# kai-neumann/OrthoSfM

Measured on AMD Instinct MI355X. Metric: image-pairs matched/sec + BA iterations/sec (N images, M tracks) at 1/2/4/8 GPU, higher is better.
Workload: dtype i8; 1 GPU; 50 orthographic images, 20000 SIFT features/img, exhaustive matching (1225 pairs, low-res gate + two-way + cross-check + lists; SURVEY 8d's unit of work: up to, not including, RANSAC-F -- the pass through RANSAC-F is `with_geometric_verification`); views=50, features_per_view=20000, pairs=1225

## Files before the change

### orthosfm_amd/csrc/match_all.hip

```cpp
#include <algorithm>
#include <chrono>
#include <cstdlib>
#include <cstring>

#include "match_internal.h"
#include "ransac_kernels.h"
#include "ransac_affine.h"

namespace osfm {

namespace {

struct Lap {
    std::chrono::steady_clock::time_point t_chunk = std::chrono::steady_clock::now();
    void operator()(const char *what) const
    {
        static const bool trace = getenv("OSFM_MATCH_TRACE") != nullptr;
        if (trace) fprintf(stderr, "[osfm match] %-18s %9.3f ms\n", what,
            std::chrono::duration<double, std::milli>(std::chrono::steady_clock::now() - t_chunk).count());
    }
};

struct ChunkLists {
    std::vector<int64_t> m12_off, corr_off;
    std::vector<int32_t> len12;
    std::vector<uint8_t> keep;
};

int compact_chunk(osfm_matcher *m, const ChunkLists &h, int n, int64_t chunk_corr, int32_t *corr, int64_t written, int *chunk_no)
{
    const osfm_match_options &o = m->opts;
    hipStream_t s = m->stream;
    OSFM_RETURN_IF(m->d_m12_off.reserve(n * 8));
    OSFM_RETURN_IF(m->d_corr_off.reserve(n * 8));
    OSFM_RETURN_IF(m->d_len12.reserve(n * 4));
    OSFM_RETURN_IF(m->d_keep_pair.reserve(n));
    const int cb = o.geometric_verification ? 0 : ((*chunk_no)++ & 1);
    DeviceBuffer &dcorr = cb ? m->d_corr_alt : m->d_corr;
    if (m->copied_used[cb]) OSFM_HIP_CHECK(hipEventSynchronize(m->ev_copied[cb]));
    OSFM_RETURN_IF(dcorr.reserve((size_t)chunk_corr * 8));
    OSFM_HIP_CHECK(hipMemcpyAsync(m->d_m12_off.ptr, h.m12_off.data(), n * 8, hipMemcpyHostToDevice, s));
    OSFM_HIP_CHECK(hipMemcpyAsync(m->d_corr_off.ptr, h.corr_off.data(), n * 8, hipMemcpyHostToDevice, s));
    OSFM_HIP_CHECK(hipMemcpyAsync(m->d_len12.ptr, h.len12.data(), n * 4, hipMemcpyHostToDevice, s));
    OSFM_HIP_CHECK(hipMemcpyAsync(m->d_keep_pair.ptr, h.keep.data(), n, hipMemcpyHostToDevice, s));
    launch_compact_pairs(n, m->out.as<int32_t>(), m->d_m12_off.as<int64_t>(),
        m->d_len12.as<int32_t>(), m->d_corr_off.as<int64_t>(), m->d_keep_pair.as<uint8_t>(),
        dcorr.as<int32_t>(), s);
    OSFM_HIP_CHECK(hipGetLastError());
    if (!o.geometric_verification) {
        OSFM_HIP_CHECK(hipEventRecord(m->ev_compact[cb], s));
        OSFM_HIP_CHECK(hipStreamWaitEvent(m->copy_stream, m->ev_compact[cb], 0));
        OSFM_HIP_CHECK(hipMemcpyAsync(corr + 2 * written, dcorr.ptr, (size_t)chunk_corr * 8,
            hipMemcpyDeviceToHost, m->copy_stream));
        OSFM_HIP_CHECK(hipEventRecord(m->ev_copied[cb], m->copy_stream));
        m->copied_used[cb] = true;
    }
    return OSFM_OK;
}

int verify_chunk(osfm_matcher *m, const osfm_pair *pairs, const int *idx, int n, const std::vector<int32_t> &counts,
    const ChunkLists &h, int64_t chunk_corr, osfm_pair_result *results, int32_t *corr, int64_t capacity,
    int64_t *written_out, bool *overflow, const Lap &lap)
{
    const osfm_match_options &o = m->opts;
    hipStream_t s = m->stream;
    std::vector<RansacJob> jobs;
    std::vector<int> job_pair;
    OSFM_RETURN_IF(m->d_inl.reserve((size_t)chunk_corr * 4));
    OSFM_RETURN_IF(m->d_inl_count.reserve((size_t)n * 4));
    for (int k = 0; k < n; ++k) {
        if (!h.keep[k]) continue;
        const int p = idx[k];
        const ViewData &a = m->views[pairs[p].view_1], &b = m->views[pairs[p].view_2];
        if (a.n_positions < 0 || b.n_positions < 0) {
            set_error("match_all: geometric verification needs osfm_match_set_positions for views %d and %d",
                pairs[p].view_1, pairs[p].view_2);
            return OSFM_E_STATE;
        }
        RansacJob j;
        memset(&j, 0, sizeof(j));
        j.pos1 = a.positions.as<float>(); j.pos2 = b.positions.as<float>();
        j.corr = m->d_corr.as<int32_t>() + 2 * h.corr_off[k];
        j.k = counts[k];
        const int64_t hi = std::max(pairs[p].view_1, pairs[p].view_2), lo = std::min(pairs[p].view_1, pairs[p].view_2);
// ... 81 lines not shown
        if (o.use_lowres_matching && np1 * np2 > 1000000) lowres_idx.push_back(p);
        else full_idx.push_back(p);
    }

    {
        const int bs = batch_size_for(m->views, o, true);
        std::vector<osfm_pair> chunk;
        for (size_t start = 0; start < lowres_idx.size(); start += bs) {
            const size_t end = std::min(lowres_idx.size(), start + bs);
            chunk.clear();
            for (size_t k = start; k < end; ++k) chunk.push_back(pairs[lowres_idx[k]]);
            BatchResult res;
            BatchMode mode;
            mode.limit = o.num_lowres_features; mode.lowres = true; mode.apply = false;
            OSFM_RETURN_IF(run_batch(m, chunk.data(), (int)chunk.size(), mode, &res));
            for (size_t k = start; k < end; ++k) {
                const int p = lowres_idx[k];
                results[p].lowres_matches = res.counts[k - start];
                if (res.counts[k - start] < o.min_lowres_matches)
                    results[p].status = OSFM_PAIR_REJECTED_LOWRES;
                else
                    full_idx.push_back(p);
            }
        }
        std::sort(full_idx.begin(), full_idx.end());
    }
    if (phase == kPhaseGate) { if (total) *total = 0; return OSFM_OK; }

    const int min_matches = std::max(8, o.min_feature_matches);
    int64_t written = 0, written_out = 0;
    bool overflow = false;
    {
        const int bs = full_batch_size(m->views, o, full_idx.size());
        int chunk_no = 0;
        std::vector<osfm_pair> chunk;
        ChunkLists h;
        for (size_t start = 0; start < full_idx.size(); start += bs) {
            const size_t end = std::min(full_idx.size(), start + bs);
            const int n = (int)(end - start);
            chunk.clear();
            for (size_t k = start; k < end; ++k) chunk.push_back(pairs[full_idx[k]]);
            const Lap lap{};
            BatchResult res;
            BatchMode full_mode;
            if (m->expect_pairs > 0)
                full_mode.expect = std::min<int>(full_batch_size(m->views, o, (size_t)m->expect_pairs), m->expect_pairs);
            OSFM_RETURN_IF(run_batch(m, chunk.data(), n, full_mode, &res));
            lap("matched");
            h.m12_off.assign(n, 0); h.corr_off.assign(n, 0); h.len12.assign(n, 0); h.keep.assign(n, 0);
            int64_t chunk_corr = 0;
            for (int k = 0; k < n; ++k) {
                const int p = full_idx[start + k];
                osfm_pair_result &r = results[p];
                r.num_matches = res.counts[k];
                if (res.counts[k] < min_matches) { r.status = OSFM_PAIR_REJECTED_COUNT; continue; }
                r.status = OSFM_PAIR_MATCHED;
                r.offset = written + chunk_corr;
                h.keep[k] = 1;
                h.m12_off[k] = res.plans[k].off12;
                h.len12[k] = res.plans[k].len12;
                h.corr_off[k] = chunk_corr;
                chunk_corr += res.counts[k];
            }
            if (!o.geometric_verification && written + chunk_corr > capacity) overflow = true;
            if (chunk_corr > 0 && (o.geometric_verification || !overflow))
                OSFM_RETURN_IF(compact_chunk(m, h, n, chunk_corr, corr, written, &chunk_no));
            if (o.geometric_verification && chunk_corr > 0)
                OSFM_RETURN_IF(verify_chunk(m, pairs, full_idx.data() + start, n, res.counts, h, chunk_corr, results, corr,
                    capacity, &written_out, &overflow, lap));
            written += chunk_corr;
        }
    }
    if (!o.geometric_verification) OSFM_HIP_CHECK(hipStreamSynchronize(m->copy_stream));
    if (o.geometric_verification) written = written_out;
    if (total) *total = written;
    if (overflow) {
        set_error("match_all: %lld correspondences need more than the given capacity %lld",
            (long long)written, (long long)capacity);
        return OSFM_E_CAPACITY;
    }
    return OSFM_OK;
}

}
```

### orthosfm_amd/csrc/match_batch.hip

```cpp
#include <algorithm>
#include <cstdlib>
#include <cstring>

#include "match_internal.h"
#include "cashash_kernels.h"

namespace osfm {

int check_view(const osfm_matcher *m, int v, const char *what) { return check_view(m->views, v, what); }

void reset_stats(osfm_matcher *m) { memset(&m->stats, 0, sizeof(m->stats)); }

int run_batch(osfm_matcher *m, const osfm_pair *pairs, int num_pairs, const BatchMode &mode,
    BatchResult *res)
{
    const bool cascade = cascade_batch(m->opts, mode);
    if (cascade) OSFM_RETURN_IF(ensure_cashash(m));
    static const int forced_seg_tiles = [] { const char *e = getenv("OSFM_SEG_TILES"); return e ? atoi(e) : 0; }();
    const char *rescan_env = getenv("OSFM_FINISH_RESCAN");
    PlanKnobs knobs;
    knobs.seg_tiles = forced_seg_tiles;
    knobs.rescan_wave = rescan_env && strcmp(rescan_env, "wave") == 0;
    BatchPlan &plan = m->plan;
    res->counts.assign(num_pairs, 0);
    OSFM_RETURN_IF(plan_batch(m->views, m->opts, m->special_max, knobs, pairs, num_pairs, mode, &plan));
    res->plans = plan.plans;
    res->out_ints = plan.out_ints;
    const std::vector<PairPlan> &plans = plan.plans;
    std::vector<MatchProblem> *probs = plan.probs;
    const std::vector<SpecialJob> &spjobs = plan.spjobs, &spjobs_wide = plan.spjobs_wide;
    const int64_t out_ints = plan.out_ints, total_queries = plan.total_queries, rs_buckets = plan.rs_buckets;
    const int *total_blocks = plan.total_blocks, *max_n = plan.max_n;

    double grow = 1.0;
    if (mode.expect > num_pairs && num_pairs > 0) grow = 1.02 * (double)mode.expect / num_pairs;
    auto grown = [&](int64_t n) { return (size_t)((double)std::max<int64_t>(n, 1) * std::max(grow, 1.0)); };
    OSFM_RETURN_IF(m->out.reserve(grown(std::max<int64_t>(out_ints, 4)) * 4));
    OSFM_RETURN_IF(m->rowparts.reserve(grown(plan.rowpart_recs) * sizeof(RowPart)));
    OSFM_RETURN_IF(m->colparts.reserve(grown(plan.colpart_recs) * sizeof(ColPart)));
    OSFM_RETURN_IF(m->keep.reserve(grown(std::max<int64_t>(plan.keep_bytes, 16))));
    OSFM_RETURN_IF(m->exact_items.reserve(grown(total_queries) * sizeof(ExactItem)));
    OSFM_RETURN_IF(m->exact_count.reserve(16));
    if (plan.bucketed) {
        OSFM_RETURN_IF(m->rs_count.reserve(grown(rs_buckets) * sizeof(int32_t)));
        OSFM_RETURN_IF(m->rs_items.reserve(grown(plan.rs_items) * sizeof(RescoreItem)));
    }
    OSFM_RETURN_IF(m->sp_parts.reserve((size_t)std::max<int64_t>(plan.sp_recs, 1) * sizeof(RowPart)));
    hipStream_t s = m->stream;
    {
        std::vector<uint8_t> seen(m->views.size(), 0);
        for (int p = 0; p < num_pairs; ++p)
            for (int v : {plans[p].v1, plans[p].v2})
                if (!seen[v]) { seen[v] = 1; if (m->views[v].ready) OSFM_HIP_CHECK(hipStreamWaitEvent(s, m->views[v].ready, 0)); }
    }
    OSFM_RETURN_IF(m->sp_col.reserve((size_t)std::max<int64_t>(plan.sp_cols, 1) * 4));
    OSFM_RETURN_IF(m->d_spjobs.reserve(std::max<size_t>(spjobs.size() + spjobs_wide.size(), 1) * sizeof(SpecialJob)));
    if (!spjobs.empty())
        OSFM_HIP_CHECK(hipMemcpyAsync(m->d_spjobs.ptr, spjobs.data(), spjobs.size() * sizeof(SpecialJob),
            hipMemcpyHostToDevice, s));
    if (!spjobs_wide.empty())
        OSFM_HIP_CHECK(hipMemcpyAsync(m->d_spjobs.as<SpecialJob>() + spjobs.size(), spjobs_wide.data(),
            spjobs_wide.size() * sizeof(SpecialJob), hipMemcpyHostToDevice, s));
    int32_t *d_out = m->out.as<int32_t>();
    OSFM_HIP_CHECK(hipMemsetAsync(d_out, 0xff, (size_t)std::max<int64_t>(out_ints, 4) * 4, s));

    OSFM_HIP_CHECK(hipMemsetAsync(m->exact_count.ptr, 0, 16, s));
    bool timed[2] = {false, false};
    bool probed = false;
    for (int type = 0; type < 2; ++type) {
        const int np = (int)probs[type].size();
        if (np == 0) continue;
        for (int i = 0; i < np; ++i) {
            probs[type][i].m12 = d_out + plan.m12_off[type][i];
            probs[type][i].m21 = d_out + plan.m21_off[type][i];
        }
        OSFM_RETURN_IF(m->d_problems[type].reserve(np * sizeof(MatchProblem)));
        OSFM_RETURN_IF(m->mark_off[type].reserve(np * 2 * sizeof(int64_t)));
        OSFM_RETURN_IF(m->counts[type].reserve(np * sizeof(int32_t)));
        OSFM_HIP_CHECK(hipMemcpyAsync(m->d_problems[type].ptr, probs[type].data(),
            np * sizeof(MatchProblem), hipMemcpyHostToDevice, s));
        OSFM_HIP_CHECK(hipMemcpyAsync(m->mark_off[type].ptr, plan.mark_off[type].data(),
            np * 2 * sizeof(int64_t), hipMemcpyHostToDevice, s));
        OSFM_HIP_CHECK(hipMemsetAsync(m->counts[type].ptr, 0, np * sizeof(int32_t), s));
        const MatchProblem *dp = m->d_problems[type].as<MatchProblem>();
        const LoweTable tab = type == 0 ? m->tab_sift : m->tab_surf;
        const int ecap = (int)std::min<int64_t>(total_queries, 0x7fffffff);
        int32_t *ecount = m->exact_count.as<int32_t>() + type;

        if (cascade) {
            OSFM_HIP_CHECK(hipEventRecord(m->ev[type][0], s));
            timed[type] = true;
            OSFM_RETURN_IF(m->cas_state.reserve((size_t)std::max<int64_t>(plan.cas_queries[type], 1) * kCasMaxCand * 4));
            launch_cashash_match(type == 0 ? 128 : 64, dp, np, max_n[type], m->cas_state.as<int32_t>(), tab, s);
            OSFM_HIP_CHECK(hipEventRecord(m->ev[type][1], s));
        } else {
            if (total_blocks[type] > 0) { OSFM_HIP_CHECK(hipEventRecord(m->ev[type][0], s)); timed[type] = true; }
            unsigned long long *probe = nullptr;
            if (type == 0 && mode.limit == 0) {
                OSFM_RETURN_IF(m->clock_probe.reserve(16));
                OSFM_HIP_CHECK(hipMemsetAsync(m->clock_probe.ptr, 0, 16, s));
                probe = m->clock_probe.as<unsigned long long>();
                probed = true;
            }
            if (!m->zero_tile.ptr) {
                OSFM_RETURN_IF(m->zero_tile.reserve((size_t)kTileCols * 128));
                OSFM_HIP_CHECK(hipMemsetAsync(m->zero_tile.ptr, 0, (size_t)kTileCols * 128, s));
            }
            launch_match_tiles(type == 0 ? 8 : 4, plan.needs_mask[type], plan.any_special[type], plan.any_c0[type],
                plan.any_corrected[type], dp, np, total_blocks[type],
                m->rowparts.as<RowPart>(), m->colparts.as<ColPart>(), s, probe, m->zero_tile.as<int8_t>());
            if (timed[type]) OSFM_HIP_CHECK(hipEventRecord(m->ev[type][1], s));
            if (type == 0 && !(spjobs.empty() && spjobs_wide.empty())) {
                OSFM_HIP_CHECK(hipEventRecord(m->ev_sp[0], s));
                launch_match_special(dp, m->d_spjobs.as<SpecialJob>(), (int)spjobs.size(), m->sp_parts.as<RowPart>(),
                    m->sp_col.as<int32_t>(), s);
                launch_match_special_wide(dp, m->d_spjobs.as<SpecialJob>() + spjobs.size(), (int)spjobs_wide.size(),
                    m->sp_parts.as<RowPart>(), m->sp_col.as<int32_t>(), s);
                OSFM_HIP_CHECK(hipEventRecord(m->ev_sp[1], s));
            }
            const bool rs = type == 0 && plan.bucketed;
            if (rs) OSFM_HIP_CHECK(hipMemsetAsync(m->rs_count.ptr, 0, (size_t)rs_buckets * sizeof(int32_t), s));
            launch_match_finish(dp, np, max_n[type], m->rowparts.as<RowPart>(),
                m->colparts.as<ColPart>(), m->sp_parts.as<RowPart>(), m->sp_col.as<int32_t>(), tab, 0,
                m->exact_items.as<ExactItem>(), ecount, ecap, rs ? m->rs_count.as<int32_t>() : nullptr,
                rs ? m->rs_items.as<RescoreItem>() : nullptr, s);
            if (rs)
                launch_match_rescore(dp, np, m->rs_count.as<int32_t>(), m->rs_items.as<RescoreItem>(), rs_buckets, tab,
                    m->exact_items.as<ExactItem>(), ecount, ecap, s);
            launch_exact_scan(type == 0 ? 128 : 64, dp, m->exact_items.as<ExactItem>(), ecount, ecap,
                tab, s);
        }
        launch_cross_check_mark(dp, np, max_n[type], m->keep.as<uint8_t>(), m->keep.as<uint8_t>(),
            m->mark_off[type].as<int64_t>(), m->counts[type].as<int32_t>(), s);
        if (mode.apply)
            launch_cross_check_apply(dp, np, max_n[type], m->keep.as<uint8_t>(),
                m->keep.as<uint8_t>(), m->mark_off[type].as<int64_t>(), s);
        OSFM_HIP_CHECK(hipGetLastError());
    }

    std::vector<int32_t> hc[2];
    int32_t hexact[4] = {0, 0, 0, 0};
    for (int type = 0; type < 2; ++type) {
        hc[type].resize(probs[type].size());
        if (!hc[type].empty())
            OSFM_HIP_CHECK(hipMemcpyAsync(hc[type].data(), m->counts[type].ptr,
                hc[type].size() * sizeof(int32_t), hipMemcpyDeviceToHost, s));
    }
    OSFM_HIP_CHECK(hipMemcpyAsync(hexact, m->exact_count.ptr, 16, hipMemcpyDeviceToHost, s));
    unsigned long long hprobe[2] = {0, 0};
    if (probed) OSFM_HIP_CHECK(hipMemcpyAsync(hprobe, m->clock_probe.ptr, 16, hipMemcpyDeviceToHost, s));
    OSFM_HIP_CHECK(hipStreamSynchronize(s));
    m->stats.tile_shader_cycles += (double)hprobe[0];
    m->stats.tile_refclk_ticks += (double)hprobe[1];
    for (int p = 0; p < num_pairs; ++p) {
        int c = 0;
        for (int type = 0; type < 2; ++type)
            if (plans[p].prob_index[type] >= 0) c += hc[type][plans[p].prob_index[type]];
        res->counts[p] = c;
    }
    for (int type = 0; type < 2; ++type) {
        if (!timed[type]) continue;
        float ms = 0.f;
        OSFM_HIP_CHECK(hipEventElapsedTime(&ms, m->ev[type][0], m->ev[type][1]));
        if (cascade) {
            m->stats.cashash_kernel_ms += ms;
            m->stats.cashash_kernel_launches += 1;
        } else if (mode.limit > 0) {
            m->stats.lowres_kernel_ms += ms;
            m->stats.lowres_kernel_launches += 1;
        } else {
            m->stats.tile_kernel_ms += ms;
            m->stats.tile_kernel_launches += 1;
            m->stats.tile_workgroups += total_blocks[type];
            if (type == 1) { m->stats.surf_tile_kernel_ms += ms; m->stats.surf_tile_kernel_launches += 1; }
        }
    }
    if (!(spjobs.empty() && spjobs_wide.empty())) {
        float ms = 0.f;
        OSFM_HIP_CHECK(hipEventElapsedTime(&ms, m->ev_sp[0], m->ev_sp[1]));
        m->stats.special_kernel_ms += ms;
        m->stats.special_kernel_launches += 1;
    }
    m->stats.exact_scan_queries += hexact[0] + hexact[1];
    if (cascade) {
    } else if (mode.limit > 0) {
        m->stats.lowres_mac_count += plan.macs;
    } else {
        m->stats.mac_count += plan.macs;
        m->stats.surf_mac_count += plan.macs_surf;
        m->stats.algorithmic_bytes += plan.alg_bytes;
    }
    return OSFM_OK;
}

}
```

### orthosfm_amd/csrc/match_internal.h

```cpp
#pragma once
#include <atomic>
#include <condition_variable>
#include <deque>
#include <functional>
#include <mutex>
#include <string>
#include <vector>

#include "match_plan.h"

struct osfm_matcher {
    int device = 0;
    hipStream_t stream = nullptr;
    osfm_match_options opts;
    std::vector<osfm::ViewData> views;
    osfm::DeviceBuffer lowe_sift, lowe_surf;
    osfm::LoweTable tab_sift, tab_surf;
    std::mutex mu;
    hipStream_t up_stream = nullptr;
    std::mutex up_mu;

    osfm::DeviceBuffer d_problems[2], rowparts, colparts, out, keep, mark_off[2], counts[2];
    osfm::DeviceBuffer exact_items, exact_count, stage_in, flags;
    osfm::DeviceBuffer rs_count, rs_items;
    osfm::DeviceBuffer sp_parts, sp_col, d_spjobs;
    osfm::DeviceBuffer clock_probe;
    osfm::BatchPlan plan;
    osfm::DeviceBuffer zero_tile;
    int special_max = 512;
    int expect_pairs = 0;
    osfm::DeviceBuffer d_m12_off, d_len12, d_corr_off, d_keep_pair, d_corr;
    osfm::DeviceBuffer d_corr_alt;
    hipStream_t copy_stream = nullptr;
    hipEvent_t ev_compact[2] = {nullptr, nullptr}, ev_copied[2] = {nullptr, nullptr};
    bool copied_used[2] = {false, false};
    osfm::DeviceBuffer d_jobs, d_inl, d_inl_count, d_corr2, d_gather_off;
    osfm::DeviceBuffer g_jobs, g_prep, g_seeds, g_u, g_m, g_list, g_out, g_off;
    hipEvent_t ev[2][2] = {{nullptr, nullptr}, {nullptr, nullptr}};
    hipEvent_t ev_sp[2] = {nullptr, nullptr};
    char *pin_ptr[2] = {nullptr, nullptr};
    size_t pin_bytes[2] = {0, 0};
    hipEvent_t pin_ev[2] = {nullptr, nullptr};
    bool pin_used[2] = {false, false};
    unsigned pin_next = 0;

    osfm::DeviceBuffer cas_proj[2], cas_sum[2], cas_avg[2], cas_state;
    std::atomic<bool> cas_dirty{true};

    osfm_match_stats stats;

    struct Staging { int32_t *ptr = nullptr; size_t ints = 0; int users = 0; };
    struct PairRequest {
        int kind;
        int v1, v2, num_features;
        int32_t *m12, *m21, *len12, *len21, *count;
        int status = OSFM_OK;
        bool done = false;
        std::string error;
        Staging *stage = nullptr;
        int64_t src12 = 0, src21 = 0;
        int32_t n12 = 0, n21 = 0;
    };
    std::vector<Staging *> comb_staging;

    std::vector<osfm_matcher *> shards;
    std::vector<Staging> shard_stage;
    std::atomic<unsigned> next_shard{0};
    std::mutex multi_mu;
    std::mutex comb_mu;
    std::condition_variable comb_cv;
    std::deque<PairRequest *> comb_queue;
    bool comb_leader = false;
};

namespace osfm {

int check_view(const osfm_matcher *m, int v, const char *what);
int run_batch(osfm_matcher *m, const osfm_pair *pairs, int num_pairs, const BatchMode &mode, BatchResult *res);
void reset_stats(osfm_matcher *m);

int upload_view(osfm_matcher *m, int view, const uint16_t *sift, int n_sift, const int16_t *surf, int n_surf);
int handoff_all(osfm_matcher *m, int view, int device, const float *d_sift, const int32_t *sift_map, int n_sift,
    const float *d_surf, const int32_t *surf_map, int n_surf, const float *d_positions,
    const std::function<int(hipStream_t)> &begin, const std::function<int(hipStream_t)> &end);
int ensure_cashash(osfm_matcher *m);

enum { kPhaseBoth = 0, kPhaseGate = 1, kPhaseFull = 2 };
int match_all_single(osfm_matcher *m, const osfm_pair *pairs, int num_pairs, osfm_pair_result *results,
    int32_t *corr, int64_t capacity, int64_t *total, int phase);

int for_each_shard(osfm_matcher *m, const std::function<int(size_t)> &fn);
int multi_match_all(osfm_matcher *m, const osfm_pair *pairs, int num_pairs, osfm_pair_result *results,
    int32_t *corr, int64_t capacity, int64_t *total);

int combine(osfm_matcher *m, osfm_matcher::PairRequest &rq);

}
```

### orthosfm_amd/csrc/match_plan.h

```cpp
#pragma once
#include <cstdint>
#include <vector>

#include "match_kernels.h"
#include "osfm_common.h"

namespace osfm {

inline int round_up(int x, int m) { return (x + m - 1) / m * m; }

struct ViewData {
    bool set = false;
    int ns = 0, nu = 0;
    int ns_pad = 0, nu_pad = 0;
    DeviceBuffer sift, sift_corr, surf, surf_corr;
    DeviceBuffer sift_raw, sift_raw_corr, special, special_corr, special_map, special_slot;
    int n_special = 0;
    int surf_norm2_max = 0;
    DeviceBuffer cas_hash[2], cas_bucket[2], cas_start[2], cas_items[2], cas_rec[2];
    DeviceBuffer positions;
    int n_positions = -1;
    hipEvent_t ready = nullptr;
    ~ViewData() { event_destroy(ready); }
    ViewData() = default;
// ... 31 lines not shown

struct PlanKnobs {
    int seg_tiles = 0;
    bool rescan_wave = false;
};

struct BatchPlan {
    std::vector<PairPlan> plans;
    std::vector<MatchProblem> probs[2];
    std::vector<int64_t> m12_off[2], m21_off[2];
    std::vector<int64_t> mark_off[2];
    std::vector<SpecialJob> spjobs, spjobs_wide;
    int64_t out_ints = 0, rowpart_recs = 0, colpart_recs = 0, keep_bytes = 0, total_queries = 0;
    int64_t sp_recs = 0, sp_cols = 0;
    int64_t rs_buckets = 0, rs_items = 0;
    int64_t cas_queries[2] = {0, 0};
    int total_blocks[2] = {0, 0}, max_n[2] = {0, 0};
    bool needs_mask[2] = {false, false};
    bool any_special[2] = {false, false};
    bool any_c0[2] = {false, false}, any_corrected[2] = {false, false};
    bool bucketed = false, cascade = false;
    int64_t macs = 0, macs_surf = 0, alg_bytes = 0;
    void clear();
};

int check_view(const std::vector<ViewData> &views, int v, const char *what);

int plan_batch(const std::vector<ViewData> &views, const osfm_match_options &opts, int special_max, const PlanKnobs &knobs,
    const osfm_pair *pairs, int num_pairs, const BatchMode &mode, BatchPlan *out);

int batch_size_for(const std::vector<ViewData> &views, const osfm_match_options &o, bool lowres);
int full_batch_size(const std::vector<ViewData> &views, const osfm_match_options &o, size_t n_full);

void deal_pairs_lpt(const std::vector<ViewData> &views, int num_shards, const osfm_pair *pairs, const std::vector<int> &cand,
    std::vector<std::vector<int>> *owner);

void build_lowe_table(float lowe, bool is_signed, std::vector<int32_t> *tab);
int max_d1_for(float dist_thres, bool is_signed);

}
```

### orthosfm_amd/csrc/match_plan.hip

```cpp
#include <algorithm>
#include <climits>
#include <cstring>
#include <queue>

#include "match_plan.h"

namespace osfm {

int check_view(const std::vector<ViewData> &views, int v, const char *what)
{
    if (v < 0 || v >= (int)views.size()) {
        set_error("%s: view id %d out of range [0, %zu)", what, v, views.size());
        return OSFM_E_ARG;
    }
    if (!views[v].set) {
        set_error("%s: view %d has not been set", what, v);
        return OSFM_E_STATE;
    }
    return OSFM_OK;
}

void BatchPlan::clear()
{
    BatchPlan fresh;
// ... 188 lines not shown
            }
            j.count = c;
        }
        for (int c = 0; c < f.nchunk; ++c) { j.chunk = c; bp.spjobs.push_back(j); }
    }
    return OSFM_OK;
}

int batch_size_for(const std::vector<ViewData> &views, const osfm_match_options &o, bool lowres)
{
    if (o.pairs_per_batch > 0) return o.pairs_per_batch;
    if (lowres) return 16384;
    size_t worst = 1;
    for (const auto &v : views) {
        const size_t n = (size_t)std::max(v.ns, v.nu) + 256;
        worst = std::max(worst, (n / kRowsPerBlock + 1) * n * sizeof(ColPart) + n * 64);
    }
    const size_t budget = (size_t)24 << 30;
    return (int)std::max<size_t>(1, std::min<size_t>(budget / worst, 4096));
}

int full_batch_size(const std::vector<ViewData> &views, const osfm_match_options &o, size_t n_full)
{
    int bs = batch_size_for(views, o, false);
    if (o.pairs_per_batch <= 0 && !o.geometric_verification && o.matcher_type != OSFM_MATCHER_CASCADE_HASHING && n_full >= 768)
        bs = std::min<int>(bs, (int)((n_full + 2) / 3));
    if (o.pairs_per_batch <= 0 && n_full > (size_t)bs) {
        const size_t parts = (n_full + bs - 1) / bs;
        bs = (int)((n_full + parts - 1) / parts);
    }
    return bs;
}

void deal_pairs_lpt(const std::vector<ViewData> &views, int num_shards, const osfm_pair *pairs, const std::vector<int> &cand,
    std::vector<std::vector<int>> *owner)
{
    const int n = num_shards;
    owner->assign(n, {});
    const int nc = (int)cand.size();
    std::vector<int64_t> w(nc);
    bool uniform = true;
    for (int i = 0; i < nc; ++i) {
        const ViewData &a = views[pairs[cand[i]].view_1], &b = views[pairs[cand[i]].view_2];
        w[i] = (int64_t)(a.ns + a.nu) * (int64_t)(b.ns + b.nu);
        uniform &= w[i] == w[0];
    }
    if (uniform) {
        for (int i = 0; i < nc; ++i) (*owner)[i % n].push_back(cand[i]);
        return;
    }
    std::vector<int> order(nc);
    for (int i = 0; i < nc; ++i) order[i] = i;
    std::stable_sort(order.begin(), order.end(), [&](int x, int y) { return w[x] > w[y]; });
    typedef std::pair<int64_t, int> Load;
    std::priority_queue<Load, std::vector<Load>, std::greater<Load>> heap;
    for (int k = 0; k < n; ++k) heap.push({0, k});
    std::vector<int> own(nc);
    for (int i : order) {
        Load l = heap.top(); heap.pop();
        own[i] = l.second;
        heap.push({l.first + w[i], l.second});
    }
    for (int i = 0; i < nc; ++i) (*owner)[own[i]].push_back(cand[i]);
}

void build_lowe_table(float lowe, bool is_signed, std::vector<int32_t> *tab)
// ... 35 lines not shown
```

Baseline: 24660 pairs/s.

## Slice post-match work of last batch and overlap compaction and D2H copy

The last full-resolution batch's post-match stage (finish, rescore, exact scan, cross-check) is split into pair slices. As each slice completes, its compaction and device-to-host correspondence copy run on the copy stream, overlapping with the remaining slices. Small per-batch uploads (problems, marks, special jobs, compaction lists) are packed into single pinned staging blocks with one memcpy each, and control counters share one memset and readback. This adds event and rescore-offset bookkeeping complexity, and the cascade path is not sliced.

```diff
diff --git a/orthosfm_amd/csrc/match_all.hip b/orthosfm_amd/csrc/match_all.hip
--- a/orthosfm_amd/csrc/match_all.hip
+++ b/orthosfm_amd/csrc/match_all.hip
@@ -27,29 +27,32 @@
     std::vector<uint8_t> keep;
 };
 
-int compact_chunk(osfm_matcher *m, const ChunkLists &h, int n, int64_t chunk_corr, int32_t *corr, int64_t written, int *chunk_no)
+int compact_chunk(osfm_matcher *m, const ChunkLists &h, int n, int64_t chunk_corr, int32_t *corr, int64_t written, int *chunk_no,
+    hipStream_t cs)
 {
     const osfm_match_options &o = m->opts;
-    hipStream_t s = m->stream;
-    OSFM_RETURN_IF(m->d_m12_off.reserve(n * 8));
-    OSFM_RETURN_IF(m->d_corr_off.reserve(n * 8));
-    OSFM_RETURN_IF(m->d_len12.reserve(n * 4));
-    OSFM_RETURN_IF(m->d_keep_pair.reserve(n));
     const int cb = o.geometric_verification ? 0 : ((*chunk_no)++ & 1);
     DeviceBuffer &dcorr = cb ? m->d_corr_alt : m->d_corr;
     if (m->copied_used[cb]) OSFM_HIP_CHECK(hipEventSynchronize(m->ev_copied[cb]));
     OSFM_RETURN_IF(dcorr.reserve((size_t)chunk_corr * 8));
-    OSFM_HIP_CHECK(hipMemcpyAsync(m->d_m12_off.ptr, h.m12_off.data(), n * 8, hipMemcpyHostToDevice, s));
-    OSFM_HIP_CHECK(hipMemcpyAsync(m->d_corr_off.ptr, h.corr_off.data(), n * 8, hipMemcpyHostToDevice, s));
-    OSFM_HIP_CHECK(hipMemcpyAsync(m->d_len12.ptr, h.len12.data(), n * 4, hipMemcpyHostToDevice, s));
-    OSFM_HIP_CHECK(hipMemcpyAsync(m->d_keep_pair.ptr, h.keep.data(), n, hipMemcpyHostToDevice, s));
-    launch_compact_pairs(n, m->out.as<int32_t>(), m->d_m12_off.as<int64_t>(),
-        m->d_len12.as<int32_t>(), m->d_corr_off.as<int64_t>(), m->d_keep_pair.as<uint8_t>(),
-        dcorr.as<int32_t>(), s);
+    const CompactLayout cl = compact_layout((size_t)n);
+    OSFM_RETURN_IF(m->d_compact[cb].reserve(cl.bytes));
+    OSFM_RETURN_IF(m->h_compact[cb].reserve(cl.bytes));
+    char *hp = m->h_compact[cb].ptr, *dp = m->d_compact[cb].as<char>();
+    memcpy(hp + cl.m12_off, h.m12_off.data(), (size_t)n * 8);
+    memcpy(hp + cl.corr_off, h.corr_off.data(), (size_t)n * 8);
+    memcpy(hp + cl.len12_off, h.len12.data(), (size_t)n * 4);
+    memcpy(hp + cl.keep_off, h.keep.data(), (size_t)n);
+    OSFM_HIP_CHECK(hipMemcpyAsync(dp, hp, cl.bytes, hipMemcpyHostToDevice, cs));
+    launch_compact_pairs(n, m->out.as<int32_t>(), reinterpret_cast<const int64_t *>(dp + cl.m12_off),
+        reinterpret_cast<const int32_t *>(dp + cl.len12_off), reinterpret_cast<const int64_t *>(dp + cl.corr_off),
+        reinterpret_cast<const uint8_t *>(dp + cl.keep_off), dcorr.as<int32_t>(), cs);
     OSFM_HIP_CHECK(hipGetLastError());
     if (!o.geometric_verification) {
-        OSFM_HIP_CHECK(hipEventRecord(m->ev_compact[cb], s));
-        OSFM_HIP_CHECK(hipStreamWaitEvent(m->copy_stream, m->ev_compact[cb], 0));
+        if (cs != m->copy_stream) {
+            OSFM_HIP_CHECK(hipEventRecord(m->ev_compact[cb], cs));
+            OSFM_HIP_CHECK(hipStreamWaitEvent(m->copy_stream, m->ev_compact[cb], 0));
+        }
         OSFM_HIP_CHECK(hipMemcpyAsync(corr + 2 * written, dcorr.ptr, (size_t)chunk_corr * 8,
             hipMemcpyDeviceToHost, m->copy_stream));
         OSFM_HIP_CHECK(hipEventRecord(m->ev_copied[cb], m->copy_stream));
@@ -197,6 +200,8 @@
     bool overflow = false;
     {
         const int bs = full_batch_size(m->views, o, full_idx.size());
+        const char *slices_env = getenv("OSFM_POST_SLICES");
+        const int post_slices_env = slices_env ? atoi(slices_env) : 0;
         int chunk_no = 0;
         std::vector<osfm_pair> chunk;
         ChunkLists h;
@@ -210,26 +215,43 @@
             BatchMode full_mode;
             if (m->expect_pairs > 0)
                 full_mode.expect = std::min<int>(full_batch_size(m->views, o, (size_t)m->expect_pairs), m->expect_pairs);
-            OSFM_RETURN_IF(run_batch(m, chunk.data(), n, full_mode, &res));
+            int64_t chunk_corr = 0;
+            auto emit = [&](int k0, int k1, hipStream_t cs) -> int {
+                const int ns = k1 - k0;
+                h.m12_off.assign(ns, 0); h.corr_off.assign(ns, 0); h.len12.assign(ns, 0); h.keep.assign(ns, 0);
+                chunk_corr = 0;
+                for (int k = k0; k < k1; ++k) {
+                    const int p = full_idx[start + k];
+                    osfm_pair_result &r = results[p];
+                    r.num_matches = res.counts[k];
+                    if (res.counts[k] < min_matches) { r.status = OSFM_PAIR_REJECTED_COUNT; continue; }
+                    r.status = OSFM_PAIR_MATCHED;
+                    r.offset = written + chunk_corr;
+                    h.keep[k - k0] = 1;
+                    h.m12_off[k - k0] = res.plans[k].off12;
+                    h.len12[k - k0] = res.plans[k].len12;
+                    h.corr_off[k - k0] = chunk_corr;
+                    chunk_corr += res.counts[k];
+                }
+                if (!o.geometric_verification && written + chunk_corr > capacity) overflow = true;
+                if (chunk_corr > 0 && (o.geometric_verification || !overflow))
+                    OSFM_RETURN_IF(compact_chunk(m, h, ns, chunk_corr, corr, written, &chunk_no, cs));
+                return OSFM_OK;
+            };
+            SliceSink sink;
+            sink.requested = post_slices_env;
+            sink.on_slice = [&](int k0, int k1) -> int {
+                OSFM_RETURN_IF(emit(k0, k1, m->copy_stream));
+                written += chunk_corr;
+                return OSFM_OK;
+            };
+            const bool last = end == full_idx.size();
+            bool sliced = false;
+            OSFM_RETURN_IF(run_batch(m, chunk.data(), n, full_mode, &res,
+                last && !o.geometric_verification ? &sink : nullptr, &sliced));
             lap("matched");
-            h.m12_off.assign(n, 0); h.corr_off.assign(n, 0); h.len12.assign(n, 0); h.keep.assign(n, 0);
-            int64_t chunk_corr = 0;
-            for (int k = 0; k < n; ++k) {
-                const int p = full_idx[start + k];
-                osfm_pair_result &r = results[p];
-                r.num_matches = res.counts[k];
-                if (res.counts[k] < min_matches) { r.status = OSFM_PAIR_REJECTED_COUNT; continue; }
-                r.status = OSFM_PAIR_MATCHED;
-                r.offset = written + chunk_corr;
-                h.keep[k] = 1;
-                h.m12_off[k] = res.plans[k].off12;
-                h.len12[k] = res.plans[k].len12;
-                h.corr_off[k] = chunk_corr;
-                chunk_corr += res.counts[k];
-            }
-            if (!o.geometric_verification && written + chunk_corr > capacity) overflow = true;
-            if (chunk_corr > 0 && (o.geometric_verification || !overflow))
-                OSFM_RETURN_IF(compact_chunk(m, h, n, chunk_corr, corr, written, &chunk_no));
+            if (sliced) continue;
+            OSFM_RETURN_IF(emit(0, n, m->stream));
             if (o.geometric_verification && chunk_corr > 0)
                 OSFM_RETURN_IF(verify_chunk(m, pairs, full_idx.data() + start, n, res.counts, h, chunk_corr, results, corr,
                     capacity, &written_out, &overflow, lap));
diff --git a/orthosfm_amd/csrc/match_batch.hip b/orthosfm_amd/csrc/match_batch.hip
--- a/orthosfm_amd/csrc/match_batch.hip
+++ b/orthosfm_amd/csrc/match_batch.hip
@@ -12,7 +12,7 @@
 void reset_stats(osfm_matcher *m) { memset(&m->stats, 0, sizeof(m->stats)); }
 
 int run_batch(osfm_matcher *m, const osfm_pair *pairs, int num_pairs, const BatchMode &mode,
-    BatchResult *res)
+    BatchResult *res, const SliceSink *sink, bool *sliced)
 {
     const bool cascade = cascade_batch(m->opts, mode);
     if (cascade) OSFM_RETURN_IF(ensure_cashash(m));
@@ -23,6 +23,7 @@
     knobs.rescan_wave = rescan_env && strcmp(rescan_env, "wave") == 0;
     BatchPlan &plan = m->plan;
     res->counts.assign(num_pairs, 0);
+    if (sliced) *sliced = false;
     OSFM_RETURN_IF(plan_batch(m->views, m->opts, m->special_max, knobs, pairs, num_pairs, mode, &plan));
     res->plans = plan.plans;
     res->out_ints = plan.out_ints;
@@ -31,6 +32,35 @@
     const std::vector<SpecialJob> &spjobs = plan.spjobs, &spjobs_wide = plan.spjobs_wide;
     const int64_t out_ints = plan.out_ints, total_queries = plan.total_queries, rs_buckets = plan.rs_buckets;
     const int *total_blocks = plan.total_blocks, *max_n = plan.max_n;
+    const int np_of[2] = {(int)probs[0].size(), (int)probs[1].size()};
+
+    std::vector<int> bounds;
+    int nslices = 1;
+    if (sink && !cascade && num_pairs > 0) nslices = post_slice_bounds(num_pairs, sink->requested, &bounds);
+    if (nslices <= 1) { bounds.assign({0, num_pairs}); nslices = 1; }
+    std::vector<int> first[2];
+    for (int type = 0; type < 2; ++type) {
+        first[type].assign(nslices + 1, np_of[type]);
+        int k = 0, seen = 0;
+        for (int p = 0; p < num_pairs; ++p) {
+            while (k < nslices && bounds[k] <= p) first[type][k++] = seen;
+            if (plans[p].prob_index[type] >= 0) ++seen;
+        }
+    }
+    std::vector<int64_t> bucket0(nslices + 1, rs_buckets), item0(nslices + 1, plan.rs_items);
+    for (int k = 0; k < nslices; ++k) {
+        const int f = first[0][k];
+        if (f < np_of[0]) { bucket0[k] = probs[0][f].rs_bucket_off; item0[k] = probs[0][f].rs_item_off; }
+    }
+    for (int k = nslices - 1; k >= 0; --k) {
+        bucket0[k] = std::min(bucket0[k], bucket0[k + 1]);
+        item0[k] = std::min(item0[k], item0[k + 1]);
+    }
+    for (int k = 1; k < nslices; ++k)
+        for (int i = first[0][k]; i < first[0][k + 1]; ++i) {
+            probs[0][i].rs_bucket_off -= bucket0[k];
+            probs[0][i].rs_item_off -= item0[k];
+        }
 
     double grow = 1.0;
     if (mode.expect > num_pairs && num_pairs > 0) grow = 1.02 * (double)mode.expect / num_pairs;
@@ -40,12 +70,14 @@
     OSFM_RETURN_IF(m->colparts.reserve(grown(plan.colpart_recs) * sizeof(ColPart)));
     OSFM_RETURN_IF(m->keep.reserve(grown(std::max<int64_t>(plan.keep_bytes, 16))));
     OSFM_RETURN_IF(m->exact_items.reserve(grown(total_queries) * sizeof(ExactItem)));
-    OSFM_RETURN_IF(m->exact_count.reserve(16));
-    if (plan.bucketed) {
-        OSFM_RETURN_IF(m->rs_count.reserve(grown(rs_buckets) * sizeof(int32_t)));
-        OSFM_RETURN_IF(m->rs_items.reserve(grown(plan.rs_items) * sizeof(RescoreItem)));
-    }
+    if (plan.bucketed) OSFM_RETURN_IF(m->rs_items.reserve(grown(plan.rs_items) * sizeof(RescoreItem)));
     OSFM_RETURN_IF(m->sp_parts.reserve((size_t)std::max<int64_t>(plan.sp_recs, 1) * sizeof(RowPart)));
+    OSFM_RETURN_IF(m->sp_col.reserve((size_t)std::max<int64_t>(plan.sp_cols, 1) * 4));
+    const ControlLayout cl = control_layout(np_of[0], np_of[1], plan.bucketed ? rs_buckets : 0);
+    const StagingLayout sl = staging_layout(np_of[0], np_of[1], spjobs.size(), spjobs_wide.size());
+    OSFM_RETURN_IF(m->d_control.reserve(grown((int64_t)cl.bytes)));
+    OSFM_RETURN_IF(m->d_batch.reserve(grown((int64_t)sl.bytes)));
+    OSFM_RETURN_IF(m->h_read.reserve(cl.read_bytes * nslices));
     hipStream_t s = m->stream;
     {
         std::vector<uint8_t> seen(m->views.size(), 0);
@@ -53,39 +85,65 @@
             for (int v : {plans[p].v1, plans[p].v2})
                 if (!seen[v]) { seen[v] = 1; if (m->views[v].ready) OSFM_HIP_CHECK(hipStreamWaitEvent(s, m->views[v].ready, 0)); }
     }
-    OSFM_RETURN_IF(m->sp_col.reserve((size_t)std::max<int64_t>(plan.sp_cols, 1) * 4));
-    OSFM_RETURN_IF(m->d_spjobs.reserve(std::max<size_t>(spjobs.size() + spjobs_wide.size(), 1) * sizeof(SpecialJob)));
-    if (!spjobs.empty())
-        OSFM_HIP_CHECK(hipMemcpyAsync(m->d_spjobs.ptr, spjobs.data(), spjobs.size() * sizeof(SpecialJob),
-            hipMemcpyHostToDevice, s));
-    if (!spjobs_wide.empty())
-        OSFM_HIP_CHECK(hipMemcpyAsync(m->d_spjobs.as<SpecialJob>() + spjobs.size(), spjobs_wide.data(),
-            spjobs_wide.size() * sizeof(SpecialJob), hipMemcpyHostToDevice, s));
     int32_t *d_out = m->out.as<int32_t>();
+    char *d_ctl = m->d_control.as<char>(), *d_up = m->d_batch.as<char>();
+
+    {
+        PinnedBlock &stage = m->h_batch;
+        OSFM_RETURN_IF(stage.reserve(sl.bytes));
+        for (int type = 0; type < 2; ++type) {
+            for (int i = 0; i < np_of[type]; ++i) {
+                probs[type][i].m12 = d_out + plan.m12_off[type][i];
+                probs[type][i].m21 = d_out + plan.m21_off[type][i];
+            }
+            if (np_of[type] == 0) continue;
+            memcpy(stage.ptr + sl.probs_off[type], probs[type].data(), (size_t)np_of[type] * sizeof(MatchProblem));
+            memcpy(stage.ptr + sl.mark_off[type], plan.mark_off[type].data(), (size_t)np_of[type] * 2 * sizeof(int64_t));
+        }
+        if (!spjobs.empty()) memcpy(stage.ptr + sl.sp_off, spjobs.data(), spjobs.size() * sizeof(SpecialJob));
+        if (!spjobs_wide.empty())
+            memcpy(stage.ptr + sl.sp_off + spjobs.size() * sizeof(SpecialJob), spjobs_wide.data(),
+                spjobs_wide.size() * sizeof(SpecialJob));
+        OSFM_HIP_CHECK(hipMemcpyAsync(d_up, stage.ptr, sl.bytes, hipMemcpyHostToDevice, s));
+    }
+    const SpecialJob *d_spjobs = reinterpret_cast<const SpecialJob *>(d_up + sl.sp_off);
     OSFM_HIP_CHECK(hipMemsetAsync(d_out, 0xff, (size_t)std::max<int64_t>(out_ints, 4) * 4, s));
-
-    OSFM_HIP_CHECK(hipMemsetAsync(m->exact_count.ptr, 0, 16, s));
+    OSFM_HIP_CHECK(hipMemsetAsync(d_ctl, 0, cl.bytes, s));
+    int32_t *d_rs_count = reinterpret_cast<int32_t *>(d_ctl + cl.rs_off);
+    const int ecap = (int)std::min<int64_t>(total_queries, 0x7fffffff);
+
+    auto post_work = [&](int type, int k) -> int {
+        const int f = first[type][k], np = first[type][k + 1] - f;
+        if (np <= 0) return OSFM_OK;
+        const MatchProblem *dp = reinterpret_cast<const MatchProblem *>(d_up + sl.probs_off[type]) + f;
+        const int64_t *d_mark = reinterpret_cast<const int64_t *>(d_up + sl.mark_off[type]) + 2 * (size_t)f;
+        int32_t *d_counts = reinterpret_cast<int32_t *>(d_ctl + cl.counts_off[type]) + f;
+        const LoweTable tab = type == 0 ? m->tab_sift : m->tab_surf;
+        int32_t *ecount = reinterpret_cast<int32_t *>(d_ctl + cl.exact_off) + type * kMaxPostSlices + k;
+        const bool rs = type == 0 && plan.bucketed;
+        int32_t *rsc = rs ? d_rs_count + bucket0[k] : nullptr;
+        RescoreItem *rsi = rs ? m->rs_items.as<RescoreItem>() + item0[k] : nullptr;
+        launch_match_finish(dp, np, max_n[type], m->rowparts.as<RowPart>(),
+            m->colparts.as<ColPart>(), m->sp_parts.as<RowPart>(), m->sp_col.as<int32_t>(), tab, 0,
+            m->exact_items.as<ExactItem>(), ecount, ecap, rsc, rsi, s);
+        if (rs)
+            launch_match_rescore(dp, np, rsc, rsi, bucket0[k + 1] - bucket0[k], tab,
+                m->exact_items.as<ExactItem>(), ecount, ecap, s);
+        launch_exact_scan(type == 0 ? 128 : 64, dp, m->exact_items.as<ExactItem>(), ecount, ecap, tab, s);
+        launch_cross_check_mark(dp, np, max_n[type], m->keep.as<uint8_t>(), m->keep.as<uint8_t>(), d_mark, d_counts, s);
+        if (mode.apply)
+            launch_cross_check_apply(dp, np, max_n[type], m->keep.as<uint8_t>(), m->keep.as<uint8_t>(), d_mark, s);
+        OSFM_HIP_CHECK(hipGetLastError());
+        return OSFM_OK;
+    };
+
     bool timed[2] = {false, false};
     bool probed = false;
     for (int type = 0; type < 2; ++type) {
-        const int np = (int)probs[type].size();
+        const int np = np_of[type];
         if (np == 0) continue;
-        for (int i = 0; i < np; ++i) {
-            probs[type][i].m12 = d_out + plan.m12_off[type][i];
-            probs[type][i].m21 = d_out + plan.m21_off[type][i];
-        }
-        OSFM_RETURN_IF(m->d_problems[type].reserve(np * sizeof(MatchProblem)));
-        OSFM_RETURN_IF(m->mark_off[type].reserve(np * 2 * sizeof(int64_t)));
-        OSFM_RETURN_IF(m->counts[type].reserve(np * sizeof(int32_t)));
-        OSFM_HIP_CHECK(hipMemcpyAsync(m->d_problems[type].ptr, probs[type].data(),
-            np * sizeof(MatchProblem), hipMemcpyHostToDevice, s));
-        OSFM_HIP_CHECK(hipMemcpyAsync(m->mark_off[type].ptr, plan.mark_off[type].data(),
-            np * 2 * sizeof(int64_t), hipMemcpyHostToDevice, s));
-        OSFM_HIP_CHECK(hipMemsetAsync(m->counts[type].ptr, 0, np * sizeof(int32_t), s));
-        const MatchProblem *dp = m->d_problems[type].as<MatchProblem>();
+        const MatchProblem *dp = reinterpret_cast<const MatchProblem *>(d_up + sl.probs_off[type]);
         const LoweTable tab = type == 0 ? m->tab_sift : m->tab_surf;
-        const int ecap = (int)std::min<int64_t>(total_queries, 0x7fffffff);
-        int32_t *ecount = m->exact_count.as<int32_t>() + type;
 
         if (cascade) {
             OSFM_HIP_CHECK(hipEventRecord(m->ev[type][0], s));
@@ -93,71 +151,79 @@
             OSFM_RETURN_IF(m->cas_state.reserve((size_t)std::max<int64_t>(plan.cas_queries[type], 1) * kCasMaxCand * 4));
             launch_cashash_match(type == 0 ? 128 : 64, dp, np, max_n[type], m->cas_state.as<int32_t>(), tab, s);
             OSFM_HIP_CHECK(hipEventRecord(m->ev[type][1], s));
-        } else {
-            if (total_blocks[type] > 0) { OSFM_HIP_CHECK(hipEventRecord(m->ev[type][0], s)); timed[type] = true; }
-            unsigned long long *probe = nullptr;
-            if (type == 0 && mode.limit == 0) {
-                OSFM_RETURN_IF(m->clock_probe.reserve(16));
-                OSFM_HIP_CHECK(hipMemsetAsync(m->clock_probe.ptr, 0, 16, s));
-                probe = m->clock_probe.as<unsigned long long>();
-                probed = true;
-            }
-            if (!m->zero_tile.ptr) {
-                OSFM_RETURN_IF(m->zero_tile.reserve((size_t)kTileCols * 128));
-                OSFM_HIP_CHECK(hipMemsetAsync(m->zero_tile.ptr, 0, (size_t)kTileCols * 128, s));
-            }
-            launch_match_tiles(type == 0 ? 8 : 4, plan.needs_mask[type], plan.any_special[type], plan.any_c0[type],
-                plan.any_corrected[type], dp, np, total_blocks[type],
-                m->rowparts.as<RowPart>(), m->colparts.as<ColPart>(), s, probe, m->zero_tile.as<int8_t>());
-            if (timed[type]) OSFM_HIP_CHECK(hipEventRecord(m->ev[type][1], s));
-            if (type == 0 && !(spjobs.empty() && spjobs_wide.empty())) {
-                OSFM_HIP_CHECK(hipEventRecord(m->ev_sp[0], s));
-                launch_match_special(dp, m->d_spjobs.as<SpecialJob>(), (int)spjobs.size(), m->sp_parts.as<RowPart>(),
-                    m->sp_col.as<int32_t>(), s);
-                launch_match_special_wide(dp, m->d_spjobs.as<SpecialJob>() + spjobs.size(), (int)spjobs_wide.size(),
-                    m->sp_parts.as<RowPart>(), m->sp_col.as<int32_t>(), s);
-                OSFM_HIP_CHECK(hipEventRecord(m->ev_sp[1], s));
-            }
-            const bool rs = type == 0 && plan.bucketed;
-            if (rs) OSFM_HIP_CHECK(hipMemsetAsync(m->rs_count.ptr, 0, (size_t)rs_buckets * sizeof(int32_t), s));
-            launch_match_finish(dp, np, max_n[type], m->rowparts.as<RowPart>(),
-                m->colparts.as<ColPart>(), m->sp_parts.as<RowPart>(), m->sp_col.as<int32_t>(), tab, 0,
-                m->exact_items.as<ExactItem>(), ecount, ecap, rs ? m->rs_count.as<int32_t>() : nullptr,
-                rs ? m->rs_items.as<RescoreItem>() : nullptr, s);
-            if (rs)
-                launch_match_rescore(dp, np, m->rs_count.as<int32_t>(), m->rs_items.as<RescoreItem>(), rs_buckets, tab,
-                    m->exact_items.as<ExactItem>(), ecount, ecap, s);
-            launch_exact_scan(type == 0 ? 128 : 64, dp, m->exact_items.as<ExactItem>(), ecount, ecap,
-                tab, s);
-        }
-        launch_cross_check_mark(dp, np, max_n[type], m->keep.as<uint8_t>(), m->keep.as<uint8_t>(),
-            m->mark_off[type].as<int64_t>(), m->counts[type].as<int32_t>(), s);
-        if (mode.apply)
-            launch_cross_check_apply(dp, np, max_n[type], m->keep.as<uint8_t>(),
-                m->keep.as<uint8_t>(), m->mark_off[type].as<int64_t>(), s);
-        OSFM_HIP_CHECK(hipGetLastError());
-    }
-
-    std::vector<int32_t> hc[2];
-    int32_t hexact[4] = {0, 0, 0, 0};
-    for (int type = 0; type < 2; ++type) {
-        hc[type].resize(probs[type].size());
-        if (!hc[type].empty())
-            OSFM_HIP_CHECK(hipMemcpyAsync(hc[type].data(), m->counts[type].ptr,
-                hc[type].size() * sizeof(int32_t), hipMemcpyDeviceToHost, s));
-    }
-    OSFM_HIP_CHECK(hipMemcpyAsync(hexact, m->exact_count.ptr, 16, hipMemcpyDeviceToHost, s));
+            launch_cross_check_mark(dp, np, max_n[type], m->keep.as<uint8_t>(), m->keep.as<uint8_t>(),
+                reinterpret_cast<const int64_t *>(d_up + sl.mark_off[type]),
+                reinterpret_cast<int32_t *>(d_ctl + cl.counts_off[type]), s);
+            if (mode.apply)
+                launch_cross_check_apply(dp, np, max_n[type], m->keep.as<uint8_t>(), m->keep.as<uint8_t>(),
+                    reinterpret_cast<const int64_t *>(d_up + sl.mark_off[type]), s);
+            OSFM_HIP_CHECK(hipGetLastError());
+            continue;
+        }
+        if (total_blocks[type] > 0) { OSFM_HIP_CHECK(hipEventRecord(m->ev[type][0], s)); timed[type] = true; }
+        unsigned long long *probe = nullptr;
+        if (type == 0 && mode.limit == 0) {
+            probe = reinterpret_cast<unsigned long long *>(d_ctl + cl.probe_off);
+            probed = true;
+        }
+        if (!m->zero_tile.ptr) {
+            OSFM_RETURN_IF(m->zero_tile.reserve((size_t)kTileCols * 128));
+            OSFM_HIP_CHECK(hipMemsetAsync(m->zero_tile.ptr, 0, (size_t)kTileCols * 128, s));
+        }
+        launch_match_tiles(type == 0 ? 8 : 4, plan.needs_mask[type], plan.any_special[type], plan.any_c0[type],
+            plan.any_corrected[type], dp, np, total_blocks[type],
+            m->rowparts.as<RowPart>(), m->colparts.as<ColPart>(), s, probe, m->zero_tile.as<int8_t>());
+        if (timed[type]) OSFM_HIP_CHECK(hipEventRecord(m->ev[type][1], s));
+        if (type == 0 && !(spjobs.empty() && spjobs_wide.empty())) {
+            OSFM_HIP_CHECK(hipEventRecord(m->ev_sp[0], s));
+            launch_match_special(dp, d_spjobs, (int)spjobs.size(), m->sp_parts.as<RowPart>(),
+                m->sp_col.as<int32_t>(), s);
+            launch_match_special_wide(dp, d_spjobs + spjobs.size(), (int)spjobs_wide.size(),
+                m->sp_parts.as<RowPart>(), m->sp_col.as<int32_t>(), s);
+            OSFM_HIP_CHECK(hipEventRecord(m->ev_sp[1], s));
+        }
+        if (nslices == 1) OSFM_RETURN_IF(post_work(type, 0));
+        else OSFM_HIP_CHECK(hipGetLastError());
+    }
+
+    const char *h_last = m->h_read.ptr + (size_t)(nslices - 1) * cl.read_bytes;
+    auto counts_of = [&](const char *h, int p0, int p1) {
+        for (int p = p0; p < p1; ++p) {
+            int c = 0;
+            for (int type = 0; type < 2; ++type)
+                if (plans[p].prob_index[type] >= 0)
+                    c += reinterpret_cast<const int32_t *>(h + cl.counts_off[type])[plans[p].prob_index[type]];
+            res->counts[p] = c;
+        }
+    };
+    if (nslices == 1) {
+        OSFM_HIP_CHECK(hipMemcpyAsync(m->h_read.ptr, d_ctl, cl.read_bytes, hipMemcpyDeviceToHost, s));
+        OSFM_HIP_CHECK(hipStreamSynchronize(s));
+        counts_of(h_last, 0, num_pairs);
+    } else {
+        for (int k = 0; k < nslices; ++k) {
+            for (int type = 0; type < 2; ++type) OSFM_RETURN_IF(post_work(type, k));
+            OSFM_RETURN_IF(m->ev_slice[k].make());
+            OSFM_HIP_CHECK(hipMemcpyAsync(m->h_read.ptr + (size_t)k * cl.read_bytes, d_ctl, cl.read_bytes,
+                hipMemcpyDeviceToHost, s));
+            OSFM_HIP_CHECK(hipEventRecord(m->ev_slice[k].e, s));
+        }
+        for (int k = 0; k < nslices; ++k) {
+            OSFM_HIP_CHECK(hipEventSynchronize(m->ev_slice[k].e));
+            counts_of(m->h_read.ptr + (size_t)k * cl.read_bytes, bounds[k], bounds[k + 1]);
+            OSFM_RETURN_IF(sink->on_slice(bounds[k], bounds[k + 1]));
+        }
+        OSFM_HIP_CHECK(hipStreamSynchronize(s));
+        if (sliced) *sliced = true;
+    }
     unsigned long long hprobe[2] = {0, 0};
-    if (probed) OSFM_HIP_CHECK(hipMemcpyAsync(hprobe, m->clock_probe.ptr, 16, hipMemcpyDeviceToHost, s));
-    OSFM_HIP_CHECK(hipStreamSynchronize(s));
+    if (probed) memcpy(hprobe, h_last + cl.probe_off, sizeof(hprobe));
+    long long hexact = 0;
+    for (int type = 0; type < 2; ++type)
+        for (int k = 0; k < nslices; ++k)
+            hexact += reinterpret_cast<const int32_t *>(h_last + cl.exact_off)[type * kMaxPostSlices + k];
     m->stats.tile_shader_cycles += (double)hprobe[0];
     m->stats.tile_refclk_ticks += (double)hprobe[1];
-    for (int p = 0; p < num_pairs; ++p) {
-        int c = 0;
-        for (int type = 0; type < 2; ++type)
-            if (plans[p].prob_index[type] >= 0) c += hc[type][plans[p].prob_index[type]];
-        res->counts[p] = c;
-    }
     for (int type = 0; type < 2; ++type) {
         if (!timed[type]) continue;
         float ms = 0.f;
@@ -175,13 +241,13 @@
             if (type == 1) { m->stats.surf_tile_kernel_ms += ms; m->stats.surf_tile_kernel_launches += 1; }
         }
     }
-    if (!(spjobs.empty() && spjobs_wide.empty())) {
+    if (!cascade && !(spjobs.empty() && spjobs_wide.empty())) {
         float ms = 0.f;
         OSFM_HIP_CHECK(hipEventElapsedTime(&ms, m->ev_sp[0], m->ev_sp[1]));
         m->stats.special_kernel_ms += ms;
         m->stats.special_kernel_launches += 1;
     }
-    m->stats.exact_scan_queries += hexact[0] + hexact[1];
+    m->stats.exact_scan_queries += hexact;
     if (cascade) {
     } else if (mode.limit > 0) {
         m->stats.lowres_mac_count += plan.macs;
diff --git a/orthosfm_amd/csrc/match_internal.h b/orthosfm_amd/csrc/match_internal.h
--- a/orthosfm_amd/csrc/match_internal.h
+++ b/orthosfm_amd/csrc/match_internal.h
@@ -8,6 +8,48 @@
 #include <vector>
 
 #include "match_plan.h"
+
+namespace osfm {
+
+struct PinnedBlock {
+    char *ptr = nullptr;
+    size_t bytes = 0;
+    PinnedBlock() = default;
+    PinnedBlock(const PinnedBlock &) = delete;
+    PinnedBlock &operator=(const PinnedBlock &) = delete;
+    ~PinnedBlock() { pinned_free(ptr, bytes); }
+    int reserve(size_t need)
+    {
+        if (need <= bytes) return OSFM_OK;
+        pinned_free(ptr, bytes);
+        ptr = nullptr; bytes = 0;
+        const size_t want = need + need / 8 + 256;
+        void *p = nullptr;
+        OSFM_HIP_CHECK(pinned_alloc(&p, want, hipHostMallocDefault));
+        ptr = static_cast<char *>(p); bytes = want;
+        return OSFM_OK;
+    }
+};
+
+struct LazyEvent {
+    hipEvent_t e = nullptr;
+    LazyEvent() = default;
+    LazyEvent(const LazyEvent &) = delete;
+    LazyEvent &operator=(const LazyEvent &) = delete;
+    ~LazyEvent() { event_destroy(e); }
+    int make()
+    {
+        if (!e) OSFM_HIP_CHECK(event_create(&e, false));
+        return OSFM_OK;
+    }
+};
+
+struct SliceSink {
+    int requested = 1;
+    std::function<int(int p0, int p1)> on_slice;
+};
+
+}
 
 struct osfm_matcher {
     int device = 0;
@@ -20,16 +62,19 @@
     hipStream_t up_stream = nullptr;
     std::mutex up_mu;
 
-    osfm::DeviceBuffer d_problems[2], rowparts, colparts, out, keep, mark_off[2], counts[2];
-    osfm::DeviceBuffer exact_items, exact_count, stage_in, flags;
-    osfm::DeviceBuffer rs_count, rs_items;
-    osfm::DeviceBuffer sp_parts, sp_col, d_spjobs;
-    osfm::DeviceBuffer clock_probe;
+    osfm::DeviceBuffer rowparts, colparts, out, keep;
+    osfm::DeviceBuffer exact_items, stage_in, flags;
+    osfm::DeviceBuffer rs_items;
+    osfm::DeviceBuffer sp_parts, sp_col;
+    osfm::DeviceBuffer d_batch, d_control;
+    osfm::PinnedBlock h_batch, h_read;
+    osfm::LazyEvent ev_slice[osfm::kMaxPostSlices];
     osfm::BatchPlan plan;
     osfm::DeviceBuffer zero_tile;
     int special_max = 512;
     int expect_pairs = 0;
-    osfm::DeviceBuffer d_m12_off, d_len12, d_corr_off, d_keep_pair, d_corr;
+    osfm::DeviceBuffer d_compact[2], d_corr;
+    osfm::PinnedBlock h_compact[2];
     osfm::DeviceBuffer d_corr_alt;
     hipStream_t copy_stream = nullptr;
     hipEvent_t ev_compact[2] = {nullptr, nullptr}, ev_copied[2] = {nullptr, nullptr};
@@ -76,7 +121,8 @@
 namespace osfm {
 
 int check_view(const osfm_matcher *m, int v, const char *what);
-int run_batch(osfm_matcher *m, const osfm_pair *pairs, int num_pairs, const BatchMode &mode, BatchResult *res);
+int run_batch(osfm_matcher *m, const osfm_pair *pairs, int num_pairs, const BatchMode &mode, BatchResult *res,
+    const SliceSink *sink = nullptr, bool *sliced = nullptr);
 void reset_stats(osfm_matcher *m);
 
 int upload_view(osfm_matcher *m, int view, const uint16_t *sift, int n_sift, const int16_t *surf, int n_surf);
diff --git a/orthosfm_amd/csrc/match_plan.h b/orthosfm_amd/csrc/match_plan.h
--- a/orthosfm_amd/csrc/match_plan.h
+++ b/orthosfm_amd/csrc/match_plan.h
@@ -87,6 +87,36 @@
 int batch_size_for(const std::vector<ViewData> &views, const osfm_match_options &o, bool lowres);
 int full_batch_size(const std::vector<ViewData> &views, const osfm_match_options &o, size_t n_full);
 
+constexpr int kMaxPostSlices = 64;
+int default_post_slices(int pairs);
+int post_slice_bounds(int pairs, int requested, std::vector<int> *bounds);
+
+struct ControlLayout {
+    size_t exact_off = 0;
+    size_t probe_off = 0;
+    size_t counts_off[2] = {0, 0};
+    size_t read_bytes = 0;
+    size_t rs_off = 0;
+    size_t bytes = 0;
+};
+ControlLayout control_layout(size_t np_sift, size_t np_surf, int64_t rs_buckets);
+
+struct StagingLayout {
+    size_t probs_off[2] = {0, 0};
+    size_t mark_off[2] = {0, 0};
+    size_t sp_off = 0;
+    size_t bytes = 0;
+};
+StagingLayout staging_layout(size_t np_sift, size_t np_surf, size_t spjobs, size_t spjobs_wide);
+
+struct CompactLayout {
+    size_t m12_off = 0, corr_off = 0;
+    size_t len12_off = 0;
+    size_t keep_off = 0;
+    size_t bytes = 0;
+};
+CompactLayout compact_layout(size_t n);
+
 void deal_pairs_lpt(const std::vector<ViewData> &views, int num_shards, const osfm_pair *pairs, const std::vector<int> &cand,
     std::vector<std::vector<int>> *owner);
 
diff --git a/orthosfm_amd/csrc/match_plan.hip b/orthosfm_amd/csrc/match_plan.hip
--- a/orthosfm_amd/csrc/match_plan.hip
+++ b/orthosfm_amd/csrc/match_plan.hip
@@ -244,6 +244,67 @@
     return bs;
 }
 
+int default_post_slices(int pairs) { return pairs >= 96 ? 3 : 1; }
+
+int post_slice_bounds(int pairs, int requested, std::vector<int> *bounds)
+{
+    bounds->clear();
+    if (pairs <= 0) return 0;
+    if (requested <= 0) requested = default_post_slices(pairs);
+    const int n = std::max(1, std::min(std::min(requested, pairs), kMaxPostSlices));
+    for (int k = 0; k <= n; ++k) bounds->push_back((int)((int64_t)pairs * k / n));
+    return n;
+}
+
+namespace {
+constexpr size_t kBlockAlign = 64;
+size_t take(size_t *at, size_t bytes)
+{
+    const size_t off = *at;
+    *at = (off + bytes + kBlockAlign - 1) / kBlockAlign * kBlockAlign;
+    return off;
+}
+}
+
+ControlLayout control_layout(size_t np_sift, size_t np_surf, int64_t rs_buckets)
+{
+    ControlLayout l;
+    size_t at = 0;
+    l.exact_off = take(&at, (size_t)2 * kMaxPostSlices * sizeof(int32_t));
+    l.probe_off = take(&at, 2 * sizeof(unsigned long long));
+    l.counts_off[0] = take(&at, np_sift * sizeof(int32_t));
+    l.counts_off[1] = take(&at, np_surf * sizeof(int32_t));
+    l.read_bytes = at;
+    l.rs_off = take(&at, (size_t)std::max<int64_t>(rs_buckets, 0) * sizeof(int32_t));
+    l.bytes = at;
+    return l;
+}
+
+StagingLayout staging_layout(size_t np_sift, size_t np_surf, size_t spjobs, size_t spjobs_wide)
+{
+    StagingLayout l;
+    size_t at = 0;
+    l.probs_off[0] = take(&at, np_sift * sizeof(MatchProblem));
+    l.probs_off[1] = take(&at, np_surf * sizeof(MatchProblem));
+    l.mark_off[0] = take(&at, np_sift * 2 * sizeof(int64_t));
+    l.mark_off[1] = take(&at, np_surf * 2 * sizeof(int64_t));
+    l.sp_off = take(&at, (spjobs + spjobs_wide) * sizeof(SpecialJob));
+    l.bytes = std::max(at, kBlockAlign);
+    return l;
+}
+
+CompactLayout compact_layout(size_t n)
+{
+    CompactLayout l;
+    size_t at = 0;
+    l.m12_off = take(&at, n * sizeof(int64_t));
+    l.corr_off = take(&at, n * sizeof(int64_t));
+    l.len12_off = take(&at, n * sizeof(int32_t));
+    l.keep_off = take(&at, n);
+    l.bytes = std::max(at, kBlockAlign);
+    return l;
+}
+
 void deal_pairs_lpt(const std::vector<ViewData> &views, int num_shards, const osfm_pair *pairs, const std::vector<int> &cand,
     std::vector<std::vector<int>> *owner)
 {
```

New measurement: 25040 pairs/s, median of 6. 1.02x the previous value.
